# AI4Science-WestlakeU/safediffcon

Measured on AMD Instinct MI355X. Metric: sampled control trajectories/sec (1000-step DDPM), higher is better.
Workload: dtype f32; 1 GPU; C4: 2D smoke Unet3D_with_Conv3D dim=64 (1,2,4) state (B,32,7,64,64), B=64 per GPU, guided 1000-step DDPM, conformal quantile on; batch_per_gpu=64, global_batch=64, step=U-Net + guidance + posterior update of the whole batch, one hipGraph replay, parallelism=batch-sharded x1, no data-path collective, conv_precision=fp32

## Files before the change

### safediffcon_amd/csrc/sdc_lablock_x3.hip

```cpp
#include "sdc_common.h"
#include "sdc_lablock_tile.h"
#include "sdc_split3.h"

namespace {

typedef __bf16 bf16x8 __attribute__((ext_vector_type(8)));
__host__ __device__ constexpr int cpitch(int C) { return C + 8; }
constexpr int PRE_CTX64 = 3, PRE_OUT64 = 1;
__device__ __forceinline__ float x3_max3(float a, float b, float c) { return fmaxf(fmaxf(a, b), c); }
__host__ __device__ constexpr int piece_e(int C) { return TT * cpitch(C); }

template <int C>
__device__ __forceinline__ void norm_tile_x3(float (&v)[C / 4], const float* __restrict__ g, int mode, float eps, float* __restrict__ xs,
                                             __bf16* __restrict__ xt, float* __restrict__ xr, float* __restrict__ red, int tid) {
    constexpr int CG = C / 4, CP = cpitch(C);
    const int tok = tid & 63, grp = tid >> 6;
    if (xr) {
#pragma unroll
        for (int k = 0; k < CG; ++k) xr[(grp * CG + k) * XP + tok] = v[k];
    }
    typedef float la_f2 __attribute__((ext_vector_type(2)));
    la_f2 s2 = {0.f, 0.f};
    float o[CG];
    if (mode == 0) {
#pragma unroll
        for (int k = 0; k < CG; k += 2) s2 += la_f2{v[k], v[k + 1]};
        red[grp * TT + tok] = s2.x + s2.y;
        __syncthreads();
        const float mean = (red[tok] + red[TT + tok] + red[2 * TT + tok] + red[3 * TT + tok]) * (1.0f / C);
        const la_f2 m2 = {mean, mean};
        la_f2 q2 = {0.f, 0.f};
#pragma unroll
        for (int k = 0; k < CG; k += 2) {
            const la_f2 d2 = la_f2{v[k], v[k + 1]} - m2;
            v[k] = d2.x; v[k + 1] = d2.y;
            q2 += d2 * d2;
        }
        red[(4 + grp) * TT + tok] = q2.x + q2.y;
        __syncthreads();
        const float var = (red[4 * TT + tok] + red[5 * TT + tok] + red[6 * TT + tok] + red[7 * TT + tok]) * (1.0f / C);
        const float rstd = rsqrtf(var + eps);
        const la_f2 r2 = {rstd, rstd};
#pragma unroll
        for (int k = 0; k < CG; k += 2) {
            const la_f2 o2 = la_f2{v[k], v[k + 1]} * r2 * la_f2{g[grp * CG + k], g[grp * CG + k + 1]};
            o[k] = o2.x; o[k + 1] = o2.y;
        }
    } else {
#pragma unroll
        for (int k = 0; k < CG; k += 2) { const la_f2 d2 = {v[k], v[k + 1]}; s2 += d2 * d2; }
        red[grp * TT + tok] = s2.x + s2.y;
        __syncthreads();
        const float nrm = sqrtf(red[tok] + red[TT + tok] + red[2 * TT + tok] + red[3 * TT + tok]);
        const float f = sqrtf((float)C) / fmaxf(nrm, 1e-12f);
        const la_f2 f2 = {f, f};
#pragma unroll
        for (int k = 0; k < CG; k += 2) {
            const la_f2 o2 = la_f2{v[k], v[k + 1]} * f2 * la_f2{g[grp * CG + k], g[grp * CG + k + 1]};
            o[k] = o2.x; o[k + 1] = o2.y;
        }
    }
    if (xs) {
#pragma unroll
        for (int k = 0; k < CG; ++k) xs[(grp * CG + k) * XP + tok] = o[k];
    }
    bf16x8* xo = reinterpret_cast<bf16x8*>(xt + tok * CP + grp * CG);
#pragma unroll
    for (int c8 = 0; c8 < CG / 8; ++c8) {
        bf16x8 ph, pm, pl;
#pragma unroll
        for (int j = 0; j < 8; ++j) {
            __bf16 h, m, l;
            split3(o[c8 * 8 + j], h, m, l);
            ph[j] = h; pm[j] = m; pl[j] = l;
        }
        xo[c8] = ph;
        xo[piece_e(C) / 8 + c8] = pm;
        xo[2 * (piece_e(C) / 8) + c8] = pl;
    }
    __syncthreads();
}

template <int C>
__device__ __forceinline__ void split_weight(const float* __restrict__ wqkv, int col, int lh, bf16x8 (&w)[3][C / 16]) {
#pragma unroll
    for (int s = 0; s < C / 16; ++s)
#pragma unroll
        for (int j = 0; j < 8; ++j) {
            __bf16 h, m, l;
            split3(wqkv[(int64_t)(16 * s + 8 * lh + j) * (3 * HID) + col], h, m, l);
            w[0][s][j] = h; w[1][s][j] = m; w[2][s][j] = l;
        }
}

template <int C, bool XA, int NPRE>
__device__ __forceinline__ void project_x3(const bf16x8 (&w)[3][C / 16], const __bf16* __restrict__ xt, int l31, int lh, f32x16 (&acc)[2]) {
    constexpr int NKS = C / 16, CP8 = cpitch(C) / 8, PE8 = piece_e(C) / 8;
    constexpr int PA[6] = {2, 1, 0, 1, 0, 0}, PB[6] = {0, 1, 2, 0, 1, 0};
#pragma unroll
    for (int r = 0; r < 16; ++r) { acc[0][r] = 0.f; acc[1][r] = 0.f; }
    const bf16x8* xp = reinterpret_cast<const bf16x8*>(xt) + l31 * CP8 + lh;
    bf16x8 xf[NPRE > 0 ? NPRE : 1][2][NKS];
#pragma unroll
    for (int p = 0; p < NPRE; ++p)
#pragma unroll
        for (int j = 0; j < 2; ++j)
#pragma unroll
            for (int s = 0; s < NKS; ++s) xf[p][j][s] = xp[p * PE8 + j * 32 * CP8 + 2 * s];
#pragma unroll
    for (int t = 0; t < 6; ++t) {
#pragma unroll
        for (int s = 0; s < NKS; ++s)
#pragma unroll
            for (int j = 0; j < 2; ++j) {
                const bf16x8 xv = PB[t] < NPRE ? xf[PB[t] < NPRE ? PB[t] : 0][j][s] : xp[PB[t] * PE8 + j * 32 * CP8 + 2 * s];
                acc[j] = XA ? __builtin_amdgcn_mfma_f32_32x32x16_bf16(xv, w[PA[t]][s], acc[j], 0, 0, 0)
                            : __builtin_amdgcn_mfma_f32_32x32x16_bf16(w[PA[t]][s], xv, acc[j], 0, 0, 0);
            }
        if (C == 64 && NPRE < 3) __builtin_amdgcn_sched_barrier(0);
    }
}

template <int C, bool GN>
__global__ __launch_bounds__(NT, (C == 64 ? 2 : 1)) SDC_NO_DS_MERGE void la_x3_ctx(const LaArgs a) {
    constexpr int NCT = C / 32;
    extern __shared__ __attribute__((aligned(16))) unsigned char smem_x3[];
    __bf16* const xt = reinterpret_cast<__bf16*>(smem_x3);
    float* const xs = reinterpret_cast<float*>(xt + 3 * piece_e(C));
    float* const red = xs + C * XP;
    float* const gcoef = red + 8 * TT;
    const int tid = threadIdx.x, lane = tid & 63, head = tid >> 6, l31 = lane & 31, lh = lane >> 5;
    const int split = blockIdx.x, seq = blockIdx.y;
    const int o = seq / a.inner, i = seq - o * a.inner;
    const float* xseq = a.x + o * a.so + i * a.si;
    const float* rseq = (GN && a.gn_res) ? a.gn_res + o * a.so + i * a.si : nullptr;
    if (GN) gn_coef_fill<C>(a.gn_stats, a.gn_gamma, a.gn_beta, a.gn_G, o, gcoef, tid);

    bf16x8 wk[3][C / 16];
    split_weight<C>(a.wqkv, HID + head * 32 + l31, lh, wk);

    f32x16 macc[NCT];
#pragma unroll
    for (int t = 0; t < NCT; ++t)
#pragma unroll
        for (int r = 0; r < 16; ++r) macc[t][r] = 0.f;
    float mrun = -INFINITY, psum = 0.f;

    const int t0 = split * a.tiles_per_split;
    const int t1 = min(t0 + a.tiles_per_split, a.ntiles);
    float xv[C / 4];
    if (t0 < t1) fetch_tile<C>(xseq + (int64_t)t0 * TT, a.sc, tid, xv);
    if (GN) __syncthreads();
    for (int tile = t0; tile < t1; ++tile) {
        if (GN) {
            gn_apply_tile<C>(xv, rseq ? rseq + (int64_t)tile * TT : nullptr, a.sc, gcoef, tid);
            float* hb = a.gn_hout + o * a.so + i * a.si + (int64_t)tile * TT;
            constexpr int CG = C / 4;
            la_gptr hp = la_uni(hb + (int64_t)(__builtin_amdgcn_readfirstlane(tid >> 6) * CG) * a.sc);
            uint32_t hoff = (uint32_t)(tid & 63) * 4u;
#pragma unroll
            for (int k = 0; k < CG; ++k) {
                asm volatile("" : "+v"(hoff));
                la_st(hp, hoff, xv[k]);
                hp += a.sc;
                asm volatile("" : "+s"(hp));
            }
        }
        norm_tile_x3<C>(xv, a.g_pre, a.pre_mode, a.eps, xs, xt, nullptr, red, tid);
        if (tile + 1 < t1) fetch_tile<C>(xseq + (int64_t)(tile + 1) * TT, a.sc, tid, xv);
        f32x16 kacc[2];
        project_x3<C, true, (C == 64 ? PRE_CTX64 : 0)>(wk, xt, l31, lh, kacc);
        float tmax = kacc[0][0];
#pragma unroll
        for (int r = 0; r < 16; ++r) tmax = x3_max3(tmax, kacc[0][r], kacc[1][r]);
        tmax = fmaxf(tmax, __shfl_xor(tmax, 32, 64));
        const float mnew = fmaxf(mrun, tmax);
        const float f = __expf(mrun - mnew);
        mrun = mnew;
        float ps = 0.f;
        const float nml = -mnew * LOG2E;
#pragma unroll
        for (int r = 0; r < 16; ++r) {
            kacc[0][r] = __builtin_amdgcn_exp2f(fmaf(kacc[0][r], LOG2E, nml));
            kacc[1][r] = __builtin_amdgcn_exp2f(fmaf(kacc[1][r], LOG2E, nml));
            ps += kacc[0][r] + kacc[1][r];
        }
        psum = psum * f + ps;
        if (__builtin_amdgcn_ballot_w64(f != 1.0f)) {
#pragma unroll
            for (int t = 0; t < NCT; ++t)
#pragma unroll
                for (int r = 0; r < 16; ++r) macc[t][r] *= f;
        }
#pragma unroll
        for (int j = 0; j < 2; ++j)
#pragma unroll
            for (int r = 0; r < 16; ++r) {
                const int tok = j * 32 + (r & 3) + 8 * (r >> 2) + 4 * lh;
#pragma unroll
                for (int t = 0; t < NCT; ++t)
                    macc[t] = __builtin_amdgcn_mfma_f32_32x32x2f32(xs[(t * 32 + l31) * XP + tok], kacc[j][r], macc[t], 0, 0, 0);
            }
        __syncthreads();
    }
    float* pp = a.part + (((int64_t)seq * a.nsplit + split) * 4 + head) * (32 * (C + 2));
#pragma unroll
    for (int t = 0; t < NCT; ++t)
#pragma unroll
        for (int r = 0; r < 16; ++r) pp[l31 * C + t * 32 + (r & 3) + 8 * (r >> 2) + 4 * lh] = macc[t][r];
    const float stot = psum + __shfl_xor(psum, 32, 64);
    if (lh == 0) { pp[32 * C + l31] = mrun; pp[32 * C + 32 + l31] = stot; }
}

template <int C>
__global__ __launch_bounds__(NT, (C == 64 ? 2 : 1)) SDC_NO_DS_MERGE void la_x3_out(const LaArgs a) {
    constexpr int NRT = C / 32;
    constexpr int TPW = NRT / 2;
    extern __shared__ __attribute__((aligned(16))) unsigned char smem_x3[];
    __bf16* const xt = reinterpret_cast<__bf16*>(smem_x3);
    float* const qs = reinterpret_cast<float*>(xt + 3 * piece_e(C));
    float* const red = qs + HID * XP;
    float* const xr = red + 8 * TT;
    float* const bg = xr + C * XP;
    const int tid = threadIdx.x, lane = tid & 63, wave = tid >> 6, l31 = lane & 31, lh = lane >> 5;
    const int seq = blockIdx.y;
    const int o = seq / a.inner, i = seq - o * a.inner;
    const float* xseq = a.x + o * a.so + i * a.si;
    float* yseq = a.y + o * a.so + i * a.si;
    const int rt = (NRT == 2) ? (wave & 1) : wave;
    const int ct0 = (NRT == 2) ? (wave >> 1) : 0;

    bf16x8 wq[3][C / 16];
    split_weight<C>(a.wqkv, wave * 32 + l31, lh, wq);
    float treg[HID / 2];
    const float* tb = a.tt + (int64_t)seq * HID * C;
#pragma unroll
    for (int ks = 0; ks < HID / 2; ++ks) treg[ks] = tb[(2 * ks + lh) * C + rt * 32 + l31];
    for (int c = tid; c < C; c += NT) {
        bg[c] = a.bo ? a.bo[c] : 0.f;
        bg[C + c] = a.g_post ? a.g_post[c] : 1.f;
    }

    const int t0 = blockIdx.x * a.tiles_per_blk;
    const int t1 = min(t0 + a.tiles_per_blk, a.ntiles);
    float xv[C / 4];
    if (t0 < t1) fetch_tile<C>(xseq + (int64_t)t0 * TT, a.sc, tid, xv);
    for (int tile = t0; tile < t1; ++tile) {
        norm_tile_x3<C>(xv, a.g_pre, a.pre_mode, a.eps, nullptr, xt, xr, red, tid);
        if (tile + 1 < t1) fetch_tile<C>(xseq + (int64_t)(tile + 1) * TT, a.sc, tid, xv);
        f32x16 qacc[2];
        project_x3<C, false, (C == 64 ? PRE_OUT64 : 0)>(wq, xt, l31, lh, qacc);
#pragma unroll
        for (int j = 0; j < 2; ++j) {
            float m = fmaxf(qacc[j][0], qacc[j][1]);
#pragma unroll
            for (int r = 2; r < 16; r += 2) m = x3_max3(m, qacc[j][r], qacc[j][r + 1]);
            m = fmaxf(m, __shfl_xor(m, 32, 64));
            typedef float la_f2 __attribute__((ext_vector_type(2)));
            const float nml = -m * LOG2E;
            const la_f2 l2 = {LOG2E, LOG2E}, n2 = {nml, nml};
            la_f2 s2 = {0.f, 0.f};
#pragma unroll
            for (int r = 0; r < 16; r += 2) {
                const la_f2 e2 = la_f2{qacc[j][r], qacc[j][r + 1]} * l2 + n2;
                const la_f2 p2 = {__builtin_amdgcn_exp2f(e2.x), __builtin_amdgcn_exp2f(e2.y)};
                qacc[j][r] = p2.x; qacc[j][r + 1] = p2.y;
                s2 += p2;
            }
            float s = s2.x + s2.y;
            s += __shfl_xor(s, 32, 64);
            const float f = 0.17677669529663687f * __builtin_amdgcn_rcpf(s);
            const la_f2 f2 = {f, f};
#pragma unroll
            for (int r = 0; r < 16; r += 2) {
                const la_f2 o2 = la_f2{qacc[j][r], qacc[j][r + 1]} * f2;
                qs[(wave * 32 + (r & 3) + 8 * (r >> 2) + 4 * lh) * XP + j * 32 + l31] = o2.x;
                qs[(wave * 32 + ((r + 1) & 3) + 8 * ((r + 1) >> 2) + 4 * lh) * XP + j * 32 + l31] = o2.y;
            }
        }
        __syncthreads();
        f32x16 yacc[TPW];
#pragma unroll
        for (int u = 0; u < TPW; ++u)
#pragma unroll
            for (int r = 0; r < 16; ++r) yacc[u][r] = bg[rt * 32 + (r & 3) + 8 * (r >> 2) + 4 * lh];
#pragma unroll
        for (int ks = 0; ks < HID / 2; ++ks)
#pragma unroll
            for (int u = 0; u < TPW; ++u)
                yacc[u] = __builtin_amdgcn_mfma_f32_32x32x2f32(treg[ks], qs[(2 * ks + lh) * XP + (ct0 + u) * 32 + l31], yacc[u], 0, 0, 0);
        if (a.post_mode >= 0) {
            float st[TPW];
#pragma unroll
            for (int u = 0; u < TPW; ++u) {
                float s = 0.f;
                if (a.post_mode == 0) {
#pragma unroll
                    for (int r = 0; r < 16; ++r) s += yacc[u][r];
                } else {
#pragma unroll
                    for (int r = 0; r < 16; ++r) s += yacc[u][r] * yacc[u][r];
                }
                s += __shfl_xor(s, 32, 64);
                if (lh == 0) red[rt * TT + (ct0 + u) * 32 + l31] = s;
            }
            __syncthreads();
#pragma unroll
            for (int u = 0; u < TPW; ++u) {
                float s = 0.f;
#pragma unroll
                for (int q = 0; q < NRT; ++q) s += red[q * TT + (ct0 + u) * 32 + l31];
                st[u] = s;
            }
            if (a.post_mode == 0) {
#pragma unroll
                for (int u = 0; u < TPW; ++u) {
                    typedef float la_f2 __attribute__((ext_vector_type(2)));
                    const float mean = st[u] * (1.0f / C);
                    const la_f2 m2 = {mean, mean};
                    la_f2 q2 = {0.f, 0.f};
#pragma unroll
                    for (int r = 0; r < 16; r += 2) {
                        const la_f2 d2 = la_f2{yacc[u][r], yacc[u][r + 1]} - m2;
                        yacc[u][r] = d2.x; yacc[u][r + 1] = d2.y;
                        q2 += d2 * d2;
                    }
                    float q = q2.x + q2.y;
                    q += __shfl_xor(q, 32, 64);
                    if (lh == 0) red[(4 + rt) * TT + (ct0 + u) * 32 + l31] = q;
                }
                __syncthreads();
#pragma unroll
                for (int u = 0; u < TPW; ++u) {
                    float q = 0.f;
#pragma unroll
                    for (int w = 0; w < NRT; ++w) q += red[(4 + w) * TT + (ct0 + u) * 32 + l31];
                    const float rstd = rsqrtf(q * (1.0f / C) + a.eps);
                    typedef float la_f2 __attribute__((ext_vector_type(2)));
                    const la_f2 r2 = {rstd, rstd};
#pragma unroll
                    for (int r = 0; r < 16; r += 2) {
                        const la_f2 o2 = la_f2{yacc[u][r], yacc[u][r + 1]} * r2 *
                                         la_f2{bg[C + rt * 32 + (r & 3) + 8 * (r >> 2) + 4 * lh], bg[C + rt * 32 + ((r + 1) & 3) + 8 * ((r + 1) >> 2) + 4 * lh]};
                        yacc[u][r] = o2.x; yacc[u][r + 1] = o2.y;
                    }
                }
            } else {
#pragma unroll
                for (int u = 0; u < TPW; ++u) {
                    const float f = sqrtf((float)C) / fmaxf(sqrtf(st[u]), 1e-12f);
#pragma unroll
                    for (int r = 0; r < 16; ++r) yacc[u][r] = yacc[u][r] * f * bg[C + rt * 32 + (r & 3) + 8 * (r >> 2) + 4 * lh];
                }
            }
        }
#pragma unroll
        for (int u = 0; u < TPW; ++u) {
            const int col = (ct0 + u) * 32 + l31;
            uint32_t loff = (uint32_t)((int64_t)(4 * lh) * a.sc + col) * 4u;
            la_gptr yrow = la_uni(yseq + (int64_t)(rt * 32) * a.sc + (int64_t)tile * TT);
            const float* xrow = xr + (rt * 32 + 4 * lh) * XP + col;
#pragma unroll
            for (int r = 0; r < 16; ++r) {
                asm volatile("" : "+v"(loff));
                la_st(yrow, loff, yacc[u][r] + xrow[((r & 3) + 8 * (r >> 2)) * XP]);
                yrow += ((r & 3) == 3 ? 5 : 1) * a.sc;
                asm volatile("" : "+s"(yrow));
            }
        }
        __syncthreads();
    }
}

size_t lds_ctx(int C) { return sizeof(__bf16) * (size_t)(3 * piece_e(C)) + sizeof(float) * (size_t)(C * XP + 8 * TT + 2 * C); }
size_t lds_out(int C) { return sizeof(__bf16) * (size_t)(3 * piece_e(C)) + sizeof(float) * (size_t)(HID * XP + 8 * TT + C * XP + 2 * C); }
static_assert((sizeof(__bf16) * 3 * piece_e(64)) % 16 == 0 && (sizeof(__bf16) * 3 * piece_e(128)) % 16 == 0, "the fp32 images start on 16 bytes");
static_assert(2 * (sizeof(__bf16) * 3 * piece_e(64) + sizeof(float) * (HID * XP + 8 * TT + 64 * XP + 2 * 64)) <= 160 * 1024, "la_x3_out<64>: two per CU");

}

namespace sdc {

int la_x3_launch_ctx(const LaArgs& a, int C, bool gn, dim3 grid, hipStream_t stream) {
    static std::atomic<uint64_t> attr0{0}, attr1{0};
    SDC_LDS_OPTIN(attr0, (la_x3_ctx<128, false>), 96 * 1024, "sdc_linattn_block");
    SDC_LDS_OPTIN(attr1, (la_x3_ctx<128, true>), 96 * 1024, "sdc_linattn_block");
    const size_t ldsb = lds_ctx(C);
    if (C == 64) {
        if (gn) hipLaunchKernelGGL((la_x3_ctx<64, true>), grid, dim3(NT), ldsb, stream, a);
        else hipLaunchKernelGGL((la_x3_ctx<64, false>), grid, dim3(NT), ldsb, stream, a);
    } else {
        if (gn) hipLaunchKernelGGL((la_x3_ctx<128, true>), grid, dim3(NT), ldsb, stream, a);
        else hipLaunchKernelGGL((la_x3_ctx<128, false>), grid, dim3(NT), ldsb, stream, a);
    }
    return SDC_OK;
}

int la_x3_launch_out(const LaArgs& a, int C, dim3 grid, hipStream_t stream) {
    static std::atomic<uint64_t> attr0{0}, attr1{0};
    SDC_LDS_OPTIN(attr0, la_x3_out<64>, 96 * 1024, "sdc_linattn_block");
    SDC_LDS_OPTIN(attr1, la_x3_out<128>, 128 * 1024, "sdc_linattn_block");
    const size_t ldsb = lds_out(C);
    if (C == 64) hipLaunchKernelGGL(la_x3_out<64>, grid, dim3(NT), ldsb, stream, a);
    else hipLaunchKernelGGL(la_x3_out<128>, grid, dim3(NT), ldsb, stream, a);
    return SDC_OK;
}

}

extern "C" int sdc_linattn_block_x3_ok(int C, int64_t n) {
    return (C == 64 && (n == 4096 || n == 2048 || n == 1024)) || (C == 128 && (n == 1024 || n == 512));
}
```

Before: 0.3049 trajectories/s.

## Replace fp32 MFMA context and output contractions with split-bf16 x3 MFMA

The context accumulation in la_x3_ctx and the output contraction in la_x3_out now use three-way bf16-split MFMA (32x32x16 bf16, six cross terms) instead of fp32 32x32x2 MFMA. Each kernel stages transposed or split bf16 images in LDS, built with DPP and perm byte shuffles during normalisation, or rebuilt from the q accumulators. The goal is to replace the slow fp32 MFMA path with the much higher-throughput bf16 path while keeping roughly fp32 accuracy. The cost is extra split/pack ALU work, different LDS footprints and limits, and an added barrier. The old paths stay reachable through a debug environment switch.

```diff
diff --git a/safediffcon_amd/csrc/sdc_lablock_x3.hip b/safediffcon_amd/csrc/sdc_lablock_x3.hip
--- a/safediffcon_amd/csrc/sdc_lablock_x3.hip
+++ b/safediffcon_amd/csrc/sdc_lablock_x3.hip
@@ -5,14 +5,23 @@
 namespace {
 
 typedef __bf16 bf16x8 __attribute__((ext_vector_type(8)));
+typedef __bf16 bf16x4 __attribute__((ext_vector_type(4)));
+typedef uint32_t u32x4 __attribute__((ext_vector_type(4)));
 __host__ __device__ constexpr int cpitch(int C) { return C + 8; }
-constexpr int PRE_CTX64 = 3, PRE_OUT64 = 1;
+constexpr int XCP = TT + 8;
+constexpr int QP = HID + 8;
+constexpr int PRE_CTX64 = 3;
+__host__ __device__ constexpr int pre_out64(bool split_y) { return split_y ? 0 : 1; }
+#define X3_TERMS constexpr int PA[6] = {2, 1, 0, 1, 0, 0}, PB[6] = {0, 1, 2, 0, 1, 0}
 __device__ __forceinline__ float x3_max3(float a, float b, float c) { return fmaxf(fmaxf(a, b), c); }
 __host__ __device__ constexpr int piece_e(int C) { return TT * cpitch(C); }
+__host__ __device__ constexpr int cpiece_e(int C) { return C * XCP; }
+constexpr int qpiece_e = TT * QP;
 
 template <int C>
 __device__ __forceinline__ void norm_tile_x3(float (&v)[C / 4], const float* __restrict__ g, int mode, float eps, float* __restrict__ xs,
-                                             __bf16* __restrict__ xt, float* __restrict__ xr, float* __restrict__ red, int tid) {
+                                             __bf16* __restrict__ xt, __bf16* __restrict__ xc, float* __restrict__ xr, float* __restrict__ red,
+                                             int tid) {
     constexpr int CG = C / 4, CP = cpitch(C);
     const int tok = tid & 63, grp = tid >> 6;
     if (xr) {
@@ -65,18 +74,32 @@
         for (int k = 0; k < CG; ++k) xs[(grp * CG + k) * XP + tok] = o[k];
     }
     bf16x8* xo = reinterpret_cast<bf16x8*>(xt + tok * CP + grp * CG);
+    const int odd = tok & 1;
+    const uint32_t sel = odd ? 0x07060302u : 0x01000504u;
+    const int ptok = (tok & ~0xD) | ((tok & 4) << 1) | ((tok & 8) >> 1);
+    uint32_t* xcw = reinterpret_cast<uint32_t*>(xc) + ((grp * CG + odd) * XCP + ptok) / 2;
 #pragma unroll
     for (int c8 = 0; c8 < CG / 8; ++c8) {
-        bf16x8 ph, pm, pl;
+        bf16x8 pv[3];
 #pragma unroll
         for (int j = 0; j < 8; ++j) {
             __bf16 h, m, l;
             split3(o[c8 * 8 + j], h, m, l);
-            ph[j] = h; pm[j] = m; pl[j] = l;
-        }
-        xo[c8] = ph;
-        xo[piece_e(C) / 8 + c8] = pm;
-        xo[2 * (piece_e(C) / 8) + c8] = pl;
+            pv[0][j] = h; pv[1][j] = m; pv[2][j] = l;
+        }
+#pragma unroll
+        for (int p = 0; p < 3; ++p) xo[p * (piece_e(C) / 8) + c8] = pv[p];
+        if (xc) {
+#pragma unroll
+            for (int p = 0; p < 3; ++p) {
+                const u32x4 w = __builtin_bit_cast(u32x4, pv[p]);
+#pragma unroll
+                for (int i = 0; i < 4; ++i) {
+                    const uint32_t nb = (uint32_t)__builtin_amdgcn_mov_dpp((int)w[i], 0xB1, 0xF, 0xF, true);
+                    xcw[p * (cpiece_e(C) / 2) + (c8 * 8 + 2 * i) * (XCP / 2)] = __builtin_amdgcn_perm(w[i], nb, sel);
+                }
+            }
+        }
     }
     __syncthreads();
 }
@@ -93,10 +116,10 @@
         }
 }
 
-template <int C, bool XA, int NPRE>
+template <int C, bool XA, int NPRE, bool MIDBAR = false>
 __device__ __forceinline__ void project_x3(const bf16x8 (&w)[3][C / 16], const __bf16* __restrict__ xt, int l31, int lh, f32x16 (&acc)[2]) {
     constexpr int NKS = C / 16, CP8 = cpitch(C) / 8, PE8 = piece_e(C) / 8;
-    constexpr int PA[6] = {2, 1, 0, 1, 0, 0}, PB[6] = {0, 1, 2, 0, 1, 0};
+    X3_TERMS;
 #pragma unroll
     for (int r = 0; r < 16; ++r) { acc[0][r] = 0.f; acc[1][r] = 0.f; }
     const bf16x8* xp = reinterpret_cast<const bf16x8*>(xt) + l31 * CP8 + lh;
@@ -117,17 +140,19 @@
                 acc[j] = XA ? __builtin_amdgcn_mfma_f32_32x32x16_bf16(xv, w[PA[t]][s], acc[j], 0, 0, 0)
                             : __builtin_amdgcn_mfma_f32_32x32x16_bf16(w[PA[t]][s], xv, acc[j], 0, 0, 0);
             }
-        if (C == 64 && NPRE < 3) __builtin_amdgcn_sched_barrier(0);
-    }
-}
-
-template <int C, bool GN>
+        if ((C == 64 && NPRE < 3) || (MIDBAR && t == 2)) __builtin_amdgcn_sched_barrier(0);
+    }
+}
+
+template <int C, bool GN, bool SPLIT_M>
 __global__ __launch_bounds__(NT, (C == 64 ? 2 : 1)) SDC_NO_DS_MERGE void la_x3_ctx(const LaArgs a) {
     constexpr int NCT = C / 32;
+    X3_TERMS;
     extern __shared__ __attribute__((aligned(16))) unsigned char smem_x3[];
     __bf16* const xt = reinterpret_cast<__bf16*>(smem_x3);
-    float* const xs = reinterpret_cast<float*>(xt + 3 * piece_e(C));
-    float* const red = xs + C * XP;
+    __bf16* const xc = xt + 3 * piece_e(C);
+    float* const xs = reinterpret_cast<float*>(xc);
+    float* const red = SPLIT_M ? reinterpret_cast<float*>(xc + 3 * cpiece_e(C)) : xs + C * XP;
     float* const gcoef = red + 8 * TT;
     const int tid = threadIdx.x, lane = tid & 63, head = tid >> 6, l31 = lane & 31, lh = lane >> 5;
     const int split = blockIdx.x, seq = blockIdx.y;
@@ -166,10 +191,10 @@
                 asm volatile("" : "+s"(hp));
             }
         }
-        norm_tile_x3<C>(xv, a.g_pre, a.pre_mode, a.eps, xs, xt, nullptr, red, tid);
+        norm_tile_x3<C>(xv, a.g_pre, a.pre_mode, a.eps, SPLIT_M ? nullptr : xs, xt, SPLIT_M ? xc : nullptr, nullptr, red, tid);
         if (tile + 1 < t1) fetch_tile<C>(xseq + (int64_t)(tile + 1) * TT, a.sc, tid, xv);
         f32x16 kacc[2];
-        project_x3<C, true, (C == 64 ? PRE_CTX64 : 0)>(wk, xt, l31, lh, kacc);
+        project_x3<C, true, (C == 64 ? PRE_CTX64 : 0), (C == 128 && SPLIT_M)>(wk, xt, l31, lh, kacc);
         float tmax = kacc[0][0];
 #pragma unroll
         for (int r = 0; r < 16; ++r) tmax = x3_max3(tmax, kacc[0][r], kacc[1][r]);
@@ -192,15 +217,40 @@
 #pragma unroll
                 for (int r = 0; r < 16; ++r) macc[t][r] *= f;
         }
-#pragma unroll
-        for (int j = 0; j < 2; ++j)
-#pragma unroll
-            for (int r = 0; r < 16; ++r) {
-                const int tok = j * 32 + (r & 3) + 8 * (r >> 2) + 4 * lh;
-#pragma unroll
-                for (int t = 0; t < NCT; ++t)
-                    macc[t] = __builtin_amdgcn_mfma_f32_32x32x2f32(xs[(t * 32 + l31) * XP + tok], kacc[j][r], macc[t], 0, 0, 0);
-            }
+        if constexpr (SPLIT_M) {
+            const bf16x8* ap = reinterpret_cast<const bf16x8*>(xc) + l31 * (XCP / 8) + lh;
+#pragma unroll
+            for (int j = 0; j < 2; ++j)
+#pragma unroll
+                for (int hf = 0; hf < 2; ++hf) {
+                    bf16x8 pb[3], af[3][NCT];
+#pragma unroll
+                    for (int e = 0; e < 8; ++e) {
+                        __bf16 h, m, l;
+                        split3(kacc[j][8 * hf + e], h, m, l);
+                        pb[0][e] = h; pb[1][e] = m; pb[2][e] = l;
+                    }
+#pragma unroll
+                    for (int p = 0; p < 3; ++p)
+#pragma unroll
+                        for (int t = 0; t < NCT; ++t) af[p][t] = ap[p * (cpiece_e(C) / 8) + t * 32 * (XCP / 8) + 4 * j + 2 * hf];
+#pragma unroll
+                    for (int k = 0; k < 6; ++k)
+#pragma unroll
+                        for (int t = 0; t < NCT; ++t)
+                            macc[t] = __builtin_amdgcn_mfma_f32_32x32x16_bf16(af[PA[k]][t], pb[PB[k]], macc[t], 0, 0, 0);
+                }
+        } else {
+#pragma unroll
+            for (int j = 0; j < 2; ++j)
+#pragma unroll
+                for (int r = 0; r < 16; ++r) {
+                    const int tok = j * 32 + (r & 3) + 8 * (r >> 2) + 4 * lh;
+#pragma unroll
+                    for (int t = 0; t < NCT; ++t)
+                        macc[t] = __builtin_amdgcn_mfma_f32_32x32x2f32(xs[(t * 32 + l31) * XP + tok], kacc[j][r], macc[t], 0, 0, 0);
+                }
+        }
         __syncthreads();
     }
     float* pp = a.part + (((int64_t)seq * a.nsplit + split) * 4 + head) * (32 * (C + 2));
@@ -212,14 +262,21 @@
     if (lh == 0) { pp[32 * C + l31] = mrun; pp[32 * C + 32 + l31] = stot; }
 }
 
-template <int C>
+__host__ __device__ constexpr size_t out_r0(int C, bool split_y) {
+    const size_t x = sizeof(__bf16) * 3 * (size_t)piece_e(C), q = sizeof(__bf16) * 3 * (size_t)qpiece_e;
+    return split_y ? (x > q ? x : q) : x;
+}
+
+template <int C, bool SPLIT_Y>
 __global__ __launch_bounds__(NT, (C == 64 ? 2 : 1)) SDC_NO_DS_MERGE void la_x3_out(const LaArgs a) {
     constexpr int NRT = C / 32;
     constexpr int TPW = NRT / 2;
+    X3_TERMS;
     extern __shared__ __attribute__((aligned(16))) unsigned char smem_x3[];
     __bf16* const xt = reinterpret_cast<__bf16*>(smem_x3);
-    float* const qs = reinterpret_cast<float*>(xt + 3 * piece_e(C));
-    float* const red = qs + HID * XP;
+    __bf16* const qt = xt;
+    float* const qs = reinterpret_cast<float*>(smem_x3 + out_r0(C, SPLIT_Y));
+    float* const red = SPLIT_Y ? qs : qs + HID * XP;
     float* const xr = red + 8 * TT;
     float* const bg = xr + C * XP;
     const int tid = threadIdx.x, lane = tid & 63, wave = tid >> 6, l31 = lane & 31, lh = lane >> 5;
@@ -232,10 +289,22 @@
 
     bf16x8 wq[3][C / 16];
     split_weight<C>(a.wqkv, wave * 32 + l31, lh, wq);
-    float treg[HID / 2];
     const float* tb = a.tt + (int64_t)seq * HID * C;
-#pragma unroll
-    for (int ks = 0; ks < HID / 2; ++ks) treg[ks] = tb[(2 * ks + lh) * C + rt * 32 + l31];
+    float treg[SPLIT_Y ? 1 : HID / 2];
+    bf16x8 tf[3][SPLIT_Y ? HID / 16 : 1];
+    if constexpr (SPLIT_Y) {
+#pragma unroll
+        for (int s = 0; s < HID / 16; ++s)
+#pragma unroll
+            for (int e = 0; e < 8; ++e) {
+                __bf16 h, m, l;
+                split3(tb[(16 * s + 8 * lh + e) * C + rt * 32 + l31], h, m, l);
+                tf[0][s][e] = h; tf[1][s][e] = m; tf[2][s][e] = l;
+            }
+    } else {
+#pragma unroll
+        for (int ks = 0; ks < HID / 2; ++ks) treg[ks] = tb[(2 * ks + lh) * C + rt * 32 + l31];
+    }
     for (int c = tid; c < C; c += NT) {
         bg[c] = a.bo ? a.bo[c] : 0.f;
         bg[C + c] = a.g_post ? a.g_post[c] : 1.f;
@@ -246,10 +315,10 @@
     float xv[C / 4];
     if (t0 < t1) fetch_tile<C>(xseq + (int64_t)t0 * TT, a.sc, tid, xv);
     for (int tile = t0; tile < t1; ++tile) {
-        norm_tile_x3<C>(xv, a.g_pre, a.pre_mode, a.eps, nullptr, xt, xr, red, tid);
+        norm_tile_x3<C>(xv, a.g_pre, a.pre_mode, a.eps, nullptr, xt, nullptr, xr, red, tid);
         if (tile + 1 < t1) fetch_tile<C>(xseq + (int64_t)(tile + 1) * TT, a.sc, tid, xv);
         f32x16 qacc[2];
-        project_x3<C, false, (C == 64 ? PRE_OUT64 : 0)>(wq, xt, l31, lh, qacc);
+        project_x3<C, false, (C == 64 ? pre_out64(SPLIT_Y) : 0)>(wq, xt, l31, lh, qacc);
 #pragma unroll
         for (int j = 0; j < 2; ++j) {
             float m = fmaxf(qacc[j][0], qacc[j][1]);
@@ -274,9 +343,31 @@
 #pragma unroll
             for (int r = 0; r < 16; r += 2) {
                 const la_f2 o2 = la_f2{qacc[j][r], qacc[j][r + 1]} * f2;
-                qs[(wave * 32 + (r & 3) + 8 * (r >> 2) + 4 * lh) * XP + j * 32 + l31] = o2.x;
-                qs[(wave * 32 + ((r + 1) & 3) + 8 * ((r + 1) >> 2) + 4 * lh) * XP + j * 32 + l31] = o2.y;
-            }
+                if constexpr (SPLIT_Y) {
+                    qacc[j][r] = o2.x; qacc[j][r + 1] = o2.y;
+                } else {
+                    qs[(wave * 32 + (r & 3) + 8 * (r >> 2) + 4 * lh) * XP + j * 32 + l31] = o2.x;
+                    qs[(wave * 32 + ((r + 1) & 3) + 8 * ((r + 1) >> 2) + 4 * lh) * XP + j * 32 + l31] = o2.y;
+                }
+            }
+        }
+        if constexpr (SPLIT_Y) {
+            __syncthreads();
+#pragma unroll
+            for (int j = 0; j < 2; ++j)
+#pragma unroll
+                for (int g4 = 0; g4 < 4; ++g4) {
+                    bf16x4 qv[3];
+#pragma unroll
+                    for (int e = 0; e < 4; ++e) {
+                        __bf16 h, m, l;
+                        split3(qacc[j][4 * g4 + e], h, m, l);
+                        qv[0][e] = h; qv[1][e] = m; qv[2][e] = l;
+                    }
+#pragma unroll
+                    for (int p = 0; p < 3; ++p)
+                        *reinterpret_cast<bf16x4*>(qt + p * qpiece_e + (j * 32 + l31) * QP + wave * 32 + 8 * g4 + 4 * lh) = qv[p];
+                }
         }
         __syncthreads();
         f32x16 yacc[TPW];
@@ -284,11 +375,28 @@
         for (int u = 0; u < TPW; ++u)
 #pragma unroll
             for (int r = 0; r < 16; ++r) yacc[u][r] = bg[rt * 32 + (r & 3) + 8 * (r >> 2) + 4 * lh];
-#pragma unroll
-        for (int ks = 0; ks < HID / 2; ++ks)
-#pragma unroll
-            for (int u = 0; u < TPW; ++u)
-                yacc[u] = __builtin_amdgcn_mfma_f32_32x32x2f32(treg[ks], qs[(2 * ks + lh) * XP + (ct0 + u) * 32 + l31], yacc[u], 0, 0, 0);
+        if constexpr (SPLIT_Y) {
+            const bf16x8* qp = reinterpret_cast<const bf16x8*>(qt) + (ct0 * 32 + l31) * (QP / 8) + lh;
+#pragma unroll
+            for (int s = 0; s < HID / 16; ++s) {
+                bf16x8 qf[3][TPW];
+#pragma unroll
+                for (int p = 0; p < 3; ++p)
+#pragma unroll
+                    for (int u = 0; u < TPW; ++u) qf[p][u] = qp[p * (qpiece_e / 8) + u * 32 * (QP / 8) + 2 * s];
+#pragma unroll
+                for (int k = 0; k < 6; ++k)
+#pragma unroll
+                    for (int u = 0; u < TPW; ++u)
+                        yacc[u] = __builtin_amdgcn_mfma_f32_32x32x16_bf16(tf[PA[k]][s], qf[PB[k]][u], yacc[u], 0, 0, 0);
+            }
+        } else {
+#pragma unroll
+            for (int ks = 0; ks < HID / 2; ++ks)
+#pragma unroll
+                for (int u = 0; u < TPW; ++u)
+                    yacc[u] = __builtin_amdgcn_mfma_f32_32x32x2f32(treg[ks], qs[(2 * ks + lh) * XP + (ct0 + u) * 32 + l31], yacc[u], 0, 0, 0);
+        }
         if (a.post_mode >= 0) {
             float st[TPW];
 #pragma unroll
@@ -372,38 +480,69 @@
     }
 }
 
-size_t lds_ctx(int C) { return sizeof(__bf16) * (size_t)(3 * piece_e(C)) + sizeof(float) * (size_t)(C * XP + 8 * TT + 2 * C); }
-size_t lds_out(int C) { return sizeof(__bf16) * (size_t)(3 * piece_e(C)) + sizeof(float) * (size_t)(HID * XP + 8 * TT + C * XP + 2 * C); }
-static_assert((sizeof(__bf16) * 3 * piece_e(64)) % 16 == 0 && (sizeof(__bf16) * 3 * piece_e(128)) % 16 == 0, "the fp32 images start on 16 bytes");
-static_assert(2 * (sizeof(__bf16) * 3 * piece_e(64) + sizeof(float) * (HID * XP + 8 * TT + 64 * XP + 2 * 64)) <= 160 * 1024, "la_x3_out<64>: two per CU");
+constexpr bool SHIP_SPLIT_M = true, SHIP_SPLIT_Y = true;
+
+constexpr size_t lds_ctx(int C, bool split_m) {
+    return sizeof(__bf16) * (size_t)(3 * piece_e(C)) + (split_m ? sizeof(__bf16) * (size_t)(3 * cpiece_e(C)) : sizeof(float) * (size_t)(C * XP)) +
+           sizeof(float) * (size_t)(8 * TT + 2 * C);
+}
+constexpr size_t lds_out(int C, bool split_y) {
+    return out_r0(C, split_y) + sizeof(float) * (size_t)((split_y ? 0 : HID * XP) + 8 * TT + C * XP + 2 * C);
+}
+static_assert((sizeof(__bf16) * 3 * piece_e(64)) % 16 == 0 && (sizeof(__bf16) * 3 * piece_e(128)) % 16 == 0, "the images behind xt start on 16 bytes");
+static_assert((sizeof(__bf16) * 3 * cpiece_e(64)) % 16 == 0 && (sizeof(__bf16) * 3 * qpiece_e) % 16 == 0, "the fp32 arrays start on 16 bytes");
+static_assert(2 * lds_ctx(64, true) <= 160 * 1024 && 2 * lds_ctx(64, false) <= 160 * 1024, "la_x3_ctx<64>: two per CU");
+static_assert(2 * lds_out(64, true) <= 160 * 1024 && 2 * lds_out(64, false) <= 160 * 1024, "la_x3_out<64>: two per CU");
+static_assert(lds_out(64, true) <= 80 * 1024 && lds_ctx(128, true) <= 112 * 1024 && lds_out(128, true) <= 128 * 1024 && lds_out(128, false) <= 128 * 1024,
+              "the LDS limits asked for below");
+
+#ifdef SDC_KERNEL_EXPERIMENTS
+int x3_dbg() { const char* v = getenv("SDC_LAX3_DBG"); return v ? atoi(v) : 0; }
+#endif
+
+template <bool SPLIT_M>
+int launch_ctx(const LaArgs& a, int C, bool gn, dim3 grid, hipStream_t stream) {
+    static std::atomic<uint64_t> attr0{0}, attr1{0};
+    SDC_LDS_OPTIN(attr0, (la_x3_ctx<128, false, SPLIT_M>), 112 * 1024, "sdc_linattn_block");
+    SDC_LDS_OPTIN(attr1, (la_x3_ctx<128, true, SPLIT_M>), 112 * 1024, "sdc_linattn_block");
+    const size_t ldsb = lds_ctx(C, SPLIT_M);
+    if (C == 64) {
+        if (gn) hipLaunchKernelGGL((la_x3_ctx<64, true, SPLIT_M>), grid, dim3(NT), ldsb, stream, a);
+        else hipLaunchKernelGGL((la_x3_ctx<64, false, SPLIT_M>), grid, dim3(NT), ldsb, stream, a);
+    } else {
+        if (gn) hipLaunchKernelGGL((la_x3_ctx<128, true, SPLIT_M>), grid, dim3(NT), ldsb, stream, a);
+        else hipLaunchKernelGGL((la_x3_ctx<128, false, SPLIT_M>), grid, dim3(NT), ldsb, stream, a);
+    }
+    return SDC_OK;
+}
+
+template <bool SPLIT_Y>
+int launch_out(const LaArgs& a, int C, dim3 grid, hipStream_t stream) {
+    static std::atomic<uint64_t> attr0{0}, attr1{0};
+    SDC_LDS_OPTIN(attr0, (la_x3_out<64, SPLIT_Y>), 96 * 1024, "sdc_linattn_block");
+    SDC_LDS_OPTIN(attr1, (la_x3_out<128, SPLIT_Y>), 128 * 1024, "sdc_linattn_block");
+    const size_t ldsb = lds_out(C, SPLIT_Y);
+    if (C == 64) hipLaunchKernelGGL((la_x3_out<64, SPLIT_Y>), grid, dim3(NT), ldsb, stream, a);
+    else hipLaunchKernelGGL((la_x3_out<128, SPLIT_Y>), grid, dim3(NT), ldsb, stream, a);
+    return SDC_OK;
+}
 
 }
 
 namespace sdc {
 
 int la_x3_launch_ctx(const LaArgs& a, int C, bool gn, dim3 grid, hipStream_t stream) {
-    static std::atomic<uint64_t> attr0{0}, attr1{0};
-    SDC_LDS_OPTIN(attr0, (la_x3_ctx<128, false>), 96 * 1024, "sdc_linattn_block");
-    SDC_LDS_OPTIN(attr1, (la_x3_ctx<128, true>), 96 * 1024, "sdc_linattn_block");
-    const size_t ldsb = lds_ctx(C);
-    if (C == 64) {
-        if (gn) hipLaunchKernelGGL((la_x3_ctx<64, true>), grid, dim3(NT), ldsb, stream, a);
-        else hipLaunchKernelGGL((la_x3_ctx<64, false>), grid, dim3(NT), ldsb, stream, a);
-    } else {
-        if (gn) hipLaunchKernelGGL((la_x3_ctx<128, true>), grid, dim3(NT), ldsb, stream, a);
-        else hipLaunchKernelGGL((la_x3_ctx<128, false>), grid, dim3(NT), ldsb, stream, a);
-    }
-    return SDC_OK;
+#ifdef SDC_KERNEL_EXPERIMENTS
+    if ((x3_dbg() & 1) == (SHIP_SPLIT_M ? 1 : 0)) return launch_ctx<!SHIP_SPLIT_M>(a, C, gn, grid, stream);
+#endif
+    return launch_ctx<SHIP_SPLIT_M>(a, C, gn, grid, stream);
 }
 
 int la_x3_launch_out(const LaArgs& a, int C, dim3 grid, hipStream_t stream) {
-    static std::atomic<uint64_t> attr0{0}, attr1{0};
-    SDC_LDS_OPTIN(attr0, la_x3_out<64>, 96 * 1024, "sdc_linattn_block");
-    SDC_LDS_OPTIN(attr1, la_x3_out<128>, 128 * 1024, "sdc_linattn_block");
-    const size_t ldsb = lds_out(C);
-    if (C == 64) hipLaunchKernelGGL(la_x3_out<64>, grid, dim3(NT), ldsb, stream, a);
-    else hipLaunchKernelGGL(la_x3_out<128>, grid, dim3(NT), ldsb, stream, a);
-    return SDC_OK;
+#ifdef SDC_KERNEL_EXPERIMENTS
+    if (((x3_dbg() >> 1) & 1) == (SHIP_SPLIT_Y ? 1 : 0)) return launch_out<!SHIP_SPLIT_Y>(a, C, grid, stream);
+#endif
+    return launch_out<SHIP_SPLIT_Y>(a, C, grid, stream);
 }
 
 }
```

Result: no change. 0.3071 trajectories/s, median of 6 (+0.7%).
